# iancze/PSOAP

Hardware: AMD Instinct MI355X
Metric: GP lnprob evals/sec (SB2, N=6000) (higher is better)
Workload: dtype f64; 1 GPU; SB2 chunk 20 epochs x 300 px (N=6000), 32 walkers per step per GPU, one chunk per GPU (BASELINE.json configs[2]; configs[3] at 8 GPUs); timed step = H2D of next proposals || eval, D2H of 32 lnprobs, gather; N=6000, components=2, walkers=32, chunks_per_gpu=1, mode=dag, stream_groups=2, parallelism=chunk-sharded x1, RCCL all_gather of walker lnprobs

## Files before the change

### include/psoap_gp.h

```cpp
#ifndef PSOAP_GP_H
#define PSOAP_GP_H

#include <stdint.h>

#ifdef __cplusplus
extern "C" {
#endif

typedef struct psoap_chunk psoap_chunk;

int psoap_version(void);
const char *psoap_last_error(void);
int psoap_device_count(int *count);

enum {
    PSOAP_SHARE_PROCS = 0,
    PSOAP_SHARE_DAG_LAUNCHES = 1,
    PSOAP_SHARE_TAINTED = 2,
    PSOAP_SHARE_RETRIES = 3,
    PSOAP_SHARE_STAGED_FALLBACKS = 4,
    PSOAP_SHARE_STAGED_POLICY = 5,
    PSOAP_SHARE_MOVED_TASKS = 6,
    PSOAP_SHARE_MOVED_XCD = 7,
    PSOAP_SHARE_LOCK_ACQUISITIONS = 8,
// ... 134 lines not shown
                       long long *tasks_per_matrix);
int psoap_stream_plan(int P, int lanes, int workers, int scheme, void *out, long long max_tasks, long long *n_tasks,
                      long long *n_slots, long long *n_ctrs, int *scheme_out);
int psoap_stream_tasklog(psoap_chunk *h, int cap, unsigned long long *out, long long max_words);
int psoap_stream_tasks(psoap_chunk *h, void *out, long long max_tasks, long long *n_tasks);

int psoap_chunk_dag_tasks(psoap_chunk *h, void *out, long long max_tasks, long long *n_tasks);

int psoap_dag_plan(int B, int P, int workers, void *out, long long max_tasks, long long *n_tasks,
                   long long *n_slots, long long *n_ctrs, unsigned int *queue_first );
int psoap_dag_plan_sky(int B, int P, const int *first, int workers, void *out, long long max_tasks, long long *n_tasks,
                       long long *n_slots, long long *n_ctrs, unsigned int *queue_first );
int psoap_sky_first(int c, int N, int B, const double *lwl, const double *gp, int *first_out, int *perm_out);
int psoap_sky_order(int c, int N, int B, const double *lwl, const double *gp, int *first_out, int *perm_out, int *cand_out);
int psoap_chunk_sky_stats(psoap_chunk *h, long long *out, int n);
int psoap_dag_plan_multi(int B, const int *Ps, int workers, void *out, long long max_tasks,
                         long long *n_tasks, long long *n_slots, long long *n_ctrs,
                         unsigned int *queue_first);
int psoap_dag_plan_aug(int P, int Mt, int Ms, int workers, int scheme, void *tasks_out,
                       long long max_tasks, long long *n_tasks, long long *n_slots,
                       long long *n_ctrs, unsigned int *queue_first);

int psoap_dag_plan_pool(int B, const int *Ps, int workers, int Mt, int Ms, int scheme, void *tasks_out,
                        long long max_tasks, long long *n_tasks, unsigned int *order_out, unsigned int *dep_out,
                        unsigned int *n_main_out, unsigned int *queue_first, int *has_pool, long long *n_ctrs);
int psoap_dag_pick_workers(int B, const int *Ps, int Mt, int compute_units, int max_workers, int *workers);

#ifdef __cplusplus
}
#endif
// ... 2 lines not shown
```

### psoap_amd/_lib.py

```python
from __future__ import annotations

import ctypes
import os

import numpy as np

from .build import LIB_PATH

_dp = ctypes.POINTER(ctypes.c_double)
_ip = ctypes.POINTER(ctypes.c_int)
_i32p = ctypes.POINTER(ctypes.c_int32)
_vp = ctypes.c_void_p

K_CLASSES = 7
K_NAMES = ("fill", "panel_update", "potrf", "trsm", "misc", "dag", "grad_contract")


class Timings(ctypes.Structure):
    _fields_ = [("ms", ctypes.c_double * K_CLASSES),
                ("launches", ctypes.c_int64 * K_CLASSES),
                ("flops", ctypes.c_double * K_CLASSES),
                ("bytes", ctypes.c_double * K_CLASSES),
                ("total_ms", ctypes.c_double)]

# ... 84 lines not shown
    "psoap_chunk_set_profiling": (ctypes.c_int, [_vp, ctypes.c_int]),
    "psoap_chunk_get_timings": (ctypes.c_int, [_vp, ctypes.POINTER(Timings)]),
    "psoap_chunk_set_stream_groups": (ctypes.c_int, [_vp, ctypes.c_int]),
    "psoap_chunk_set_mode": (ctypes.c_int, [_vp, ctypes.c_int]),
    "psoap_chunk_dag_tasklog": (ctypes.c_int, [_vp, ctypes.POINTER(ctypes.c_uint64), ctypes.c_longlong]),
    "psoap_chunk_dag_tasks": (ctypes.c_int, [_vp, _vp, ctypes.c_longlong, ctypes.POINTER(ctypes.c_longlong)]),
    "psoap_dag_plan": (ctypes.c_int, [ctypes.c_int, ctypes.c_int, ctypes.c_int, _vp, ctypes.c_longlong,
                                      ctypes.POINTER(ctypes.c_longlong), ctypes.POINTER(ctypes.c_longlong),
                                      ctypes.POINTER(ctypes.c_longlong), ctypes.POINTER(ctypes.c_uint32)]),
    "psoap_dag_plan_sky": (ctypes.c_int, [ctypes.c_int, ctypes.c_int, _ip, ctypes.c_int, _vp, ctypes.c_longlong,
                                          ctypes.POINTER(ctypes.c_longlong), ctypes.POINTER(ctypes.c_longlong),
                                          ctypes.POINTER(ctypes.c_longlong), ctypes.POINTER(ctypes.c_uint32)]),
    "psoap_sky_first": (ctypes.c_int, [ctypes.c_int, ctypes.c_int, ctypes.c_int, _dp, _dp, _ip, _ip]),
    "psoap_sky_order": (ctypes.c_int, [ctypes.c_int, ctypes.c_int, ctypes.c_int, _dp, _dp, _ip, _ip, _ip]),
    "psoap_chunk_sky_stats": (ctypes.c_int, [_vp, ctypes.POINTER(ctypes.c_longlong), ctypes.c_int]),
    "psoap_dag_plan_multi": (ctypes.c_int, [ctypes.c_int, _ip, ctypes.c_int, _vp, ctypes.c_longlong,
                                      ctypes.POINTER(ctypes.c_longlong), ctypes.POINTER(ctypes.c_longlong),
                                      ctypes.POINTER(ctypes.c_longlong), ctypes.POINTER(ctypes.c_uint32)]),
    "psoap_dag_plan_aug": (ctypes.c_int, [ctypes.c_int, ctypes.c_int, ctypes.c_int, ctypes.c_int, ctypes.c_int, _vp,
                                          ctypes.c_longlong, ctypes.POINTER(ctypes.c_longlong),
                                          ctypes.POINTER(ctypes.c_longlong), ctypes.POINTER(ctypes.c_longlong),
                                          ctypes.POINTER(ctypes.c_uint32)]),
    "psoap_dag_pick_workers": (ctypes.c_int, [ctypes.c_int, _ip, ctypes.c_int, ctypes.c_int, ctypes.c_int, _ip]),
    "psoap_dag_plan_pool": (ctypes.c_int, [ctypes.c_int, _ip, ctypes.c_int, ctypes.c_int, ctypes.c_int, ctypes.c_int, _vp,
                                           ctypes.c_longlong, ctypes.POINTER(ctypes.c_longlong), ctypes.POINTER(ctypes.c_uint32),
                                           ctypes.POINTER(ctypes.c_uint32), ctypes.POINTER(ctypes.c_uint32),
                                           ctypes.POINTER(ctypes.c_uint32), _ip, ctypes.POINTER(ctypes.c_longlong)]),
}

BENCH_SIGNATURES = {
# ... 105 lines not shown
```

### psoap_amd/chunk.py

```python
from __future__ import annotations

import ctypes

import numpy as np

from . import _lib
from ._lib import K_NAMES, Timings, as_f64, check, dptr


class ChunkHandle:
    def __init__(self, fl, sigma, max_batch: int = 1, device: int | None = None):
        self._L = _lib.load()
        self.fl = as_f64(fl)
        self.sigma = as_f64(sigma, self.fl.shape)
        if self.fl.ndim != 1:
            raise ValueError("fl and sigma must be 1-D")
        self.N = int(self.fl.shape[0])
        self.max_batch = int(max_batch)
        self.device = _lib.default_device() if device is None else int(device)
        self._h = ctypes.c_void_p()
        check(self._L.psoap_chunk_create(ctypes.byref(self._h), self.device, self.N, dptr(self.fl),
                                         dptr(self.sigma), self.max_batch), "psoap_chunk_create")
        self._B = 0
        self.n_epochs = 0
# ... 245 lines not shown
        t = Timings()
        check(self._L.psoap_chunk_get_timings(self._h, ctypes.byref(t)), "psoap_chunk_get_timings")
        out = {"total_ms": t.total_ms}
        for k, name in enumerate(K_NAMES):
            out[name] = {"ms": t.ms[k], "launches": int(t.launches[k]), "flops": t.flops[k], "bytes": t.bytes[k]}
        return out

    def sky_stats(self) -> dict:
        names = ("tiles_planned", "tiles_dense", "units_planned", "units_dense", "plan_builds", "cache_hits", "skyline_on")
        out = (ctypes.c_longlong * len(names))()
        n = self._L.psoap_chunk_sky_stats(self._h, out, len(names))
        if n != len(names):
            raise _lib.PsoapError(f"psoap_chunk_sky_stats reports {n} fields, psoap_amd.chunk names {len(names)}")
        return dict(zip(names, (int(v) for v in out)))


class StreamPipeline:

    def __init__(self, handle: ChunkHandle, c: int, walkers: int, groups: int = 2, scheme: int = -1, submit=None):
        if walkers % groups:
            raise ValueError("walkers must be a multiple of groups")
        self.h, self.c, self.walkers, self.groups = handle, int(c), int(walkers), int(groups)
        self.rows = [slice(g * walkers // groups, (g + 1) * walkers // groups) for g in range(groups)]
        handle.stream_open(c, walkers, scheme)
        self._submit = submit if submit is not None else handle.stream_submit
        self.tickets = [None] * groups
        self.period = None

    def _go(self, g, arrays, mu_GP):
        r = self.rows[g]
# ... 109 lines not shown
```

### psoap_amd/csrc/dag_kernel.hpp

```cpp
#pragma once
#include "dag_task.hpp"

#include "chol_kernels.hpp"
#include "fill_kernels.hpp"
#include "potrf_blocked.hpp"
#include "potrf_spine.hpp"
#include "orbit_kernels.hpp"

namespace psoap {

struct alignas(64) MatFlags {
    int rows_done;
    int potrf_done;
    int cnt[2];
    int next_done;
    int off1_ready;
    int step_w[4];
    int cnt3;
    int pad[5];
    int xcol[256][2];
    int rvrow[256];
};
static_assert(sizeof(MatFlags) == 64 + 2048 + 1024, "one cache line of row state + the per-column progress words");

// ... 152 lines not shown
    int* cnt = M3 ? (q % 3 == 2 ? &f->cnt3 : &f->cnt[q % 3]) : &f->cnt[q & 1];
    const int old = __hip_atomic_fetch_add(cnt, n, PSOAP_RLX_AGENT);
    if (old + n == ntasks_row) {
        __builtin_amdgcn_fence(__ATOMIC_ACQ_REL, "agent");
        asm volatile("s_waitcnt vmcnt(0)" ::: "memory");
        __hip_atomic_store(cnt, 0, PSOAP_RLX_AGENT);
        asm volatile("s_waitcnt vmcnt(0)" ::: "memory");
        if (ctl && q > 0) dag_spin_ge(&f->rows_done, q, ctl, 11u);
        __hip_atomic_store(&f->rows_done, q + 1, __ATOMIC_RELEASE, __HIP_MEMORY_SCOPE_AGENT);
    }
}

template <bool SW = false, class SM = SmemKernel, bool ROWMAP = false, bool TD = false>
__device__ __forceinline__ void dag_update(Tile& t, double* Km, int ld, int k0, int j0, int pa, int pb, MatFlags* f,
                                           DagCtl* ctl, bool wait_next, unsigned long long* tl, int wave_s = -1, SM sm = SM(),
                                           int* wa = nullptr, int* wb = nullptr)
{
    if (pb <= pa) return;
    const bool diag = (k0 == j0);
    unsigned long long w0 = 0;
    if (tl && threadIdx.x == 0) w0 = __builtin_amdgcn_s_memrealtime();
    if (pb - pa > 1) {
        if constexpr (TD) dag_wait_ge2(wa, wb, pb - 1, ctl, 1u);
        else dag_wait_ge(&f->rows_done, pb - 1, ctl, 1u);
        if (tl && threadIdx.x == 0) {
            const unsigned long long w1 = __builtin_amdgcn_s_memrealtime();
            tl[7] += (w1 - w0) << 40;
        }
        const size_t r0 = (size_t)pa * NB;
        tile_gemm_tn<SW, SM, ROWMAP>(t, Km + r0 * ld + k0, (size_t)ld, Km + r0 * ld + j0, (size_t)ld, (pb - 1 - pa) * NB, diag, 0x7fffffff, wave_s, sm);
    }
    if (tl && threadIdx.x == 0) w0 = __builtin_amdgcn_s_memrealtime();
    if constexpr (TD) dag_wait_ge2(wa, wb, pb, ctl, 2u);
    else dag_wait_ge(wait_next ? &f->next_done : &f->rows_done, pb, ctl, 2u);
    if (tl && threadIdx.x == 0) {
        const unsigned long long w1 = __builtin_amdgcn_s_memrealtime();
        tl[4] = w1;
        tl[7] += (w1 - w0) << 40;
    }
    const size_t r1 = (size_t)(pb - 1) * NB;
    tile_gemm_tn<SW, SM, ROWMAP>(t, Km + r1 * ld + k0, (size_t)ld, Km + r1 * ld + j0, (size_t)ld, NB, diag, 0x7fffffff, wave_s, sm);
}

template <class SM>
__device__ __forceinline__ void dag_update_following(Tile& t, const double* __restrict__ A, const double* __restrict__ B,
                                                     size_t ld, int* xa, int* xb, int base, unsigned int* err, int wave, SM sm,
                                                     unsigned long long* tl = nullptr)
{
    const int wr = wave >> 1, wc = wave & 1;
    const int lane = hw_lane();
    int avail = ps::x_wait(xa, xb, base, err, 1, lane);
    if (tl && threadIdx.x == 0) tl[4] = __builtin_amdgcn_s_memrealtime();
    __builtin_amdgcn_fence(__ATOMIC_ACQUIRE, "agent");
    stage_glds_w(A, ld, B, ld, 0, 0, wave, sm);
    __syncthreads();
#pragma unroll 1
// ... 25 lines not shown
    const double* rowx;
    const double* diag;
    double* S;
    size_t lds;
};

struct DagMat {
    double* K;
    double* R;
    double* Wt;
    const double* lw;
    const double* gp;
    const double* sigma;
    MatAcc* acc;
    int N, Npad, P, ld;
};

#ifdef PSOAP_FAST_STREAM
#define DAG_FAST_STORE(stream) true
#else
#define DAG_FAST_STORE(stream) (!(stream))
#endif
template <int C, bool AUG, bool INPLACE = false, bool ROWMAP = false, bool FAST = false, bool WT = true>
__device__ __forceinline__ void dag_store_updated(Tile& t, double* __restrict__ dest, size_t ldd, int k0, int j0,
                                                  const double* __restrict__ lw, const GpDev& g, double dsum,
                                                  const double* __restrict__ sigma, int N, double scale,
                                                  int Npad, const DagAug& aug, double* __restrict__ mirror = nullptr,
                                                  bool plain = false)
{
    static_assert(INPLACE || !ROWMAP, "tiles that go to memory use the plain accumulator map");
// ... 1328 lines not shown
#else
        if (LAT && preload && ttype == DAG_DIAG && (task.type & DAG_WAITNEXT) && task.pb - task.pa == 1) {
            dag_diag_fast(Km, ld, k0, Wm, Rv, mat.acc, prev, Npad, f, ctl, q, ntasks_row, (task.type & DAG_FUSED) != 0,
                          &arrive_l[task.ctr], n_wait, dag_opaque_lds(psoap_smem), dag_opaque_lds(vec1), dag_opaque_lds(vec2),
                          tlog_l ? tlog_l + ticket * 8 : nullptr);
            dag_task_end<STREAM>(st, b, mat.acc, mat.P, where0, ctl, wave_s);
            continue;
        }
#endif
        t.zero();
        if (preload) {
            dag_wait_ge(&arrive_l[tctr], n_wait, ctl, 4u);
            dag_sub_partials<false, true>(t, prev, 1);
            n_prev = 0;
        }
        dag_update<true, SmemKernel, false, !LAT && DAG_TILE_DEPS>(
            t, Km, ld, k0, j0, task.pa, task.pb, f, ctl, ttype == DAG_DIAG && (task.type & DAG_WAITNEXT) != 0,
            tlog_l ? tlog_l + ticket * 8 : nullptr, wave_s, SmemKernel(), &f->rvrow[q], &f->rvrow[j]);
        if (tlog_l && threadIdx.x == 0) tlog_l[ticket * 8 + 5] = __builtin_amdgcn_s_memrealtime();
        if (!preload && n_wait > 0) dag_wait_ge(&arrive_l[tctr], n_wait, ctl, 4u);
        if (tlog_l && threadIdx.x == 0) tlog_l[ticket * 8 + 6] = __builtin_amdgcn_s_memrealtime();
        dag_sub_partials<false, true>(t, prev, n_prev);
        {
            GpDev g;
            load_gp(mat.gp, C, g);
            double dsum = g.a2[0];
            {
#pragma clang fp contract(off)
                for (int c = 1; c < C; ++c) dsum = dsum + g.a2[c];
            }
            double* dest = is_part ? (wspace_l + (size_t)task.slot * SLOT) : (Km + (size_t)k0 * ld + j0);
            size_t ldd = is_part ? (size_t)NB : (size_t)ld;
            double* mirror = nullptr;
// ... 82 lines not shown
```

### psoap_amd/csrc/plan_abi.hpp

```cpp
#pragma once
#include <string.h>

#include <algorithm>
#include <vector>

#include "abi_error.hpp"
#include "dag_plan.hpp"
#include "sky_rules.hpp"

using namespace psoap;

static void plan_export(const DagPlan& plan, void* out, long long max_tasks, long long* n_tasks, long long* n_slots,
                        long long* n_ctrs, unsigned int* queue_first)
{
    *n_tasks = (long long)plan.tasks.size();
    if (n_slots) *n_slots = plan.n_slots;
    if (n_ctrs) *n_ctrs = plan.n_ctrs;
    if (queue_first) memcpy(queue_first, plan.queues.first, sizeof plan.queues.first);
    if (out) {
        const long long n = max_tasks < *n_tasks ? max_tasks : *n_tasks;
        memcpy(out, plan.tasks.data(), sizeof(DagTask) * n);
    }
}

// ... 9 lines not shown
                                  long long* n_tasks, long long* n_slots, long long* n_ctrs, unsigned int* queue_first)
{
    if (B < 1 || P < 1 || P > 255 || workers < 1 || !n_tasks || !first) FAIL("psoap_dag_plan_sky: bad arguments");
    bool any = false;
    for (int j = 0; j < P; ++j) {
        if (first[j] < 0 || first[j] > (j > 0 ? j - 1 : 0) || (j > 0 && first[j] < first[j - 1]))
            FAIL("psoap_dag_plan_sky: first must be non-decreasing with 0 <= first[j] <= max(j - 1, 0)");
        any = any || first[j] > 0;
    }
    DagPlan plan = any ? dag_build_tasks(std::vector<int>((size_t)B, P), workers, 0, 0, 0, 0, first) : dag_build_tasks(B, P, workers);
    plan_export(plan, out, max_tasks, n_tasks, n_slots, n_ctrs, queue_first);
    return 0;
}

static long long sky_host_candidate(int c, int N, int B, const double* lwl, const double* gp, int cand, std::vector<int>& perm,
                                    std::vector<int>& first)
{
    const int P = round_up(N, NB) / NB;
    double w[3];
    sky_cand_weights(c, cand, w);
    std::vector<unsigned long long> key((size_t)N);
    for (int i = 0; i < N; ++i) {
        double v[3] = {0.0, 0.0, 0.0};
        for (int k = 0; k < c; ++k) v[k] = lwl[(size_t)k * N + i];
        key[i] = sky_key(sky_cand_key(c, w, v));
    }
    perm.resize((size_t)N);
    first.assign((size_t)P, 0);
    for (int i = 0; i < N; ++i) perm[i] = i;
    std::stable_sort(perm.begin(), perm.end(), [&key](int a, int b) { return key[a] < key[b]; });
    std::vector<double> x((size_t)c * N), lo((size_t)c * P), hi((size_t)c * P);
    std::vector<int> fb((size_t)P);
    for (int b = 0; b < B; ++b) {
        for (int k = 0; k < c; ++k)
            for (int r = 0; r < N; ++r) x[(size_t)k * N + r] = lwl[((size_t)b * c + k) * N + perm[r]];
        for (int k = 0; k < c; ++k)
            for (int t = 0; t < P; ++t)
                sky_interval(x.data() + (size_t)k * N, t * NB, (t + 1) * NB < N ? (t + 1) * NB : N, &lo[(size_t)k * P + t],
                             &hi[(size_t)k * P + t]);
        double p2[3] = {0.0, 0.0, 0.0};
        const bool ok = sky_gp(gp + (size_t)b * 2 * c, c, p2);
        for (int j = 0; j < P; ++j) fb[j] = sky_first_raw(j, P, c, lo.data(), hi.data(), p2, ok);
        sky_first_finish(fb.data(), P);
        for (int j = 0; j < P; ++j) first[j] = (b == 0 || fb[j] < first[j]) ? fb[j] : first[j];
    }
    return sky_cost(first.data(), P);
}

static void sky_host_order(int c, int N, int B, const double* lwl, const double* gp, int n_cand, int* first_out, int* perm_out,
                           int* cand_out)
{
    const int P = round_up(N, NB) / NB;
    std::vector<int> perm((size_t)N), first((size_t)P, 0);
    for (int i = 0; i < N; ++i) perm[i] = i;
    int best = 0;
    if (N <= SKY_MAX_N) {
        long long best_cost = sky_host_candidate(c, N, B, lwl, gp, 0, perm, first);
        std::vector<int> pk, fk;
        for (int k = 1; k < n_cand; ++k) {
            const long long cost = sky_host_candidate(c, N, B, lwl, gp, k, pk, fk);
            if (cost < best_cost) {
                best_cost = cost;
                best = k;
                perm.swap(pk);
                first.swap(fk);
            }
        }
    }
    if (perm_out) memcpy(perm_out, perm.data(), sizeof(int) * (size_t)N);
    if (first_out) memcpy(first_out, first.data(), sizeof(int) * (size_t)P);
    if (cand_out) *cand_out = best;
}

extern "C" int psoap_sky_first(int c, int N, int B, const double* lwl, const double* gp, int* first_out, int* perm_out)
{
    if (c < 1 || c > 3 || N < 1 || B < 1 || !lwl || !gp) FAIL("psoap_sky_first: bad arguments");
    sky_host_order(c, N, B, lwl, gp, 1, first_out, perm_out, nullptr);
    return 0;
}

extern "C" int psoap_sky_order(int c, int N, int B, const double* lwl, const double* gp, int* first_out, int* perm_out,
                               int* cand_out)
{
    if (c < 1 || c > 3 || N < 1 || B < 1 || !lwl || !gp) FAIL("psoap_sky_order: bad arguments");
    sky_host_order(c, N, B, lwl, gp, sky_n_cand(c), first_out, perm_out, cand_out);
    return 0;
}

extern "C" int psoap_stream_plan(int P, int lanes, int workers, int scheme, void* out, long long max_tasks,
                                 long long* n_tasks, long long* n_slots, long long* n_ctrs, int* scheme_out)
{
    if (P < 1 || P > 255 || lanes < 1 || lanes > STREAM_MAX_LANES || workers < 1 || scheme < -1 || scheme > 2 || !n_tasks)
        FAIL("psoap_stream_plan: bad arguments");
    if (scheme < 0) scheme = dag_auto_scheme(std::vector<int>((size_t)lanes, P));
    DagPlan plan = dag_build_lane_plan(P, lanes, workers, scheme);
    plan_export(plan, out, max_tasks, n_tasks, n_slots, n_ctrs, nullptr);
    if (scheme_out) *scheme_out = plan.scheme;
    return 0;
}

// ... 48 lines not shown
```

### psoap_amd/csrc/psoap_gp.hip

```cpp
#include "../../include/psoap_gp.h"

#include <math.h>
#include <stdio.h>
#include <stdlib.h>
#include <stddef.h>
#include <string.h>

#include <errno.h>
#include <time.h>
#include <unistd.h>

#include <algorithm>
#include <atomic>
#include <chrono>
#include <memory>
#include <mutex>
#include <set>
#include <string>
#include <vector>

#include "chol_kernels.hpp"
#include "dag_kernel.hpp"
#include "solo_kernel.hpp"
#include "dag_launch.hpp"
// ... 30 lines not shown
{
    char bus[64] = {0};
    return hipDeviceGetPCIBusId(bus, (int)sizeof bus, device) == hipSuccess ? std::string(bus) : std::string();
}

struct BatchSlot {
    Grow<double> dLwl;
    Grow<double> dGp;
    Grow<double> dLwlS;
    Grow<double> dFlS;
    Grow<double> dSigmaS;
    Grow<int> dPerm;
    Grow<int> dCand;
    Grow<int> dFirstB;
    Grow<int, true> hFirst;
    Grow<int> dTooFast;
    bool toofast_dirty = false;
    Grow<DagMat> dMats;
    int mats_B = 0, mats_C = 0;
    bool mats_sorted = false;
    bool sky_valid = false;
    int B = 0, C = 0;
    double mu = 1.0;
    std::vector<char> neg;
    Event evUpload;
    Event evEval;
};

namespace psoap { struct PredictWs; struct GradWs; }

// ... 44 lines not shown
    Grow<double> dWt;
    Grow<double> dR;
    Grow<MatAcc> dAcc;
    Grow<double> dVel;
    Grow<double> dOut;
    Grow<double> dDates;
    Grow<double> dPorb;
    Grow<double, true> hPorb;
    Grow<unsigned int, true> hDagErr;
    int mode = 1;
    int dag_grid = 0, n_cus = 0;
    DagWorkspace dag;
    int plan_B = 0, plan_workers = 0;
    bool sky = false;
    bool sky_order = true;
    std::vector<int> plan_first;
    DagPlanWork plan_work;
    struct SkyPlan {
        int B;
        std::vector<int> first;
        DagPlan plan;
        int workers;
        DagPlanWork work;
        Grow<DagTask> dTasks;
    };
    std::vector<SkyPlan> sky_cache;
    long long sky_stats[7] = {};
    Grow<unsigned long long> dTlog;
    long long tlog_tasks = 0;
    Grow<double, true> hLwl, hGp, hVel, hOut;
// ... 128 lines not shown
    NEED(h->dWt, nb * WT_STRIDE);
    HIP_TRY(hipMemset(h->dWt, 0, sizeof(double) * nb * WT_STRIDE));
    NEED(h->dR, nb * h->Npad);
    NEED(h->dAcc, ACC_ROWS * nb);
    NEED(h->dOut, nb);
    NEED(h->dPorb, nb * 13);
    NEED(h->hPorb, nb * 13);
    NEED(h->hLwl, nb * 3 * N);
    NEED(h->hGp, nb * 6);
    NEED(h->hOut, nb);
    {
        const char* e = getenv("PSOAP_SKYLINE");
        h->sky = N <= SKY_MAX_N && !(e && e[0] == '0');
        e = getenv("PSOAP_SKY_ORDER");
        h->sky_order = !(e && e[0] == '0');
    }
    const size_t n_cand = h->sky_order ? SKY_MAX_CAND : 1;
    for (BatchSlot& sl : h->slot) {
        if (h->sky) {
            NEED(sl.dLwlS, nb * 3 * N);
            NEED(sl.dFlS, N);
            NEED(sl.dSigmaS, N);
            NEED(sl.dPerm, n_cand * N);
            NEED(sl.dCand, 1);
            HIP_TRY(hipMemset(sl.dCand, 0, sizeof(int)));
            NEED(sl.dFirstB, n_cand * nb * h->P);
            NEED(sl.hFirst, h->P);
            memset(sl.hFirst, 0, sizeof(int) * h->P);
        }
        NEED(sl.dLwl, nb * 3 * N);
        NEED(sl.dGp, nb * 6);
        NEED(sl.dTooFast, nb);
        HIP_TRY(hipMemset(sl.dTooFast, 0, sizeof(int) * nb));
        NEED(sl.dMats, nb);
        HIP_TRY(sl.evUpload.create());
        HIP_TRY(sl.evEval.create());
    }
    const size_t tiles = nb * (size_t)h->P * (h->P + 1) / 2;
    HIP_TRY(h->dag.ctl.need(sizeof(DagCtl) + sizeof(MatFlags) * nb + sizeof(int) * (tiles + 16 + (9 * tiles + 1024) / 32 + 8)));
    NEED(h->hDagErr, 16);
    h->hDagErr[0] = 0;
    if (int rc = dag_workers(h->device, &h->dag_grid, &h->n_cus)) return rc;
// ... 111 lines not shown
    if (out) {
        const long long n = max_tasks < tasks ? max_tasks : tasks;
        HIP_TRY(hipMemcpy(out, h->dTlog, sizeof(unsigned long long) * 8 * n, hipMemcpyDeviceToHost));
    }
    return 0;
}


extern "C" int psoap_chunk_sky_stats(psoap_chunk* h, long long* out, int n)
{
    if (!h || !out || n < 0) FAIL("psoap_chunk_sky_stats: bad arguments");
    for (int i = 0; i < n && i < 7; ++i) out[i] = h->sky_stats[i];
    return 7;
}

extern "C" int psoap_chunk_dag_tasks(psoap_chunk* h, void* out, long long max_tasks, long long* n_tasks)
{
    if (!h || !n_tasks) FAIL("bad arguments");
    DEVICE_SCOPE(h->device);
    if (set_dev(h)) return 1;
    *n_tasks = h->dag.n_tasks;
    if (out && h->dag.tasks) {
        const long long n = max_tasks < (long long)h->dag.n_tasks ? max_tasks : (long long)h->dag.n_tasks;
        HIP_TRY(hipMemcpy(out, h->dag.tasks, sizeof(DagTask) * n, hipMemcpyDeviceToHost));
    }
    return 0;
}

extern "C" int psoap_chunk_set_mode(psoap_chunk* h, int mode)
{
// ... 51 lines not shown
static bool sky_batch(const psoap_chunk* h, int B)
{
    return h->mode == 1 && h->P <= 255 && !dag_fixed_plan() && dag_lnlike_scheme(std::vector<int>((size_t)B, h->P)) == 0;
}

static int upload_end(psoap_chunk* h, BatchSlot& sl)
{
    HIP_TRY(hipMemcpyAsync(sl.dGp, h->hGp, sizeof(double) * (size_t)sl.B * 2 * sl.C, hipMemcpyHostToDevice, h->copy()));
    sl.sky_valid = h->sky && sky_batch(h, sl.B);
    if (sl.sky_valid) {
        const int N = h->N, rows = sl.B * sl.C;
        hipStream_t s = h->copy();
        const int K = h->sky_order ? sky_n_cand(sl.C) : 1;
        hipLaunchKernelGGL(k_sky_perm, dim3((N + 255) / 256, K), dim3(256), 0, s, sl.dLwl, sl.C, N, sl.dPerm);
        hipLaunchKernelGGL(k_sky_first, dim3(sl.B, K), dim3(256), 0, s, sl.dLwl, sl.dPerm, sl.dGp, sl.C, N, h->P, sl.dFirstB);
        hipLaunchKernelGGL(k_sky_choose, dim3(1), dim3(256), 0, s, sl.dFirstB, sl.B, h->P, K, sl.hFirst, sl.dCand);
        hipLaunchKernelGGL(k_sky_gather, dim3((N + 255) / 256, rows + 2), dim3(256), 0, s, sl.dPerm, sl.dCand, N, rows, sl.dLwl,
                           sl.dLwlS, h->dFl, sl.dFlS, h->dSigma, sl.dSigmaS);
        HIP_TRY(hipGetLastError());
    }
    HIP_TRY(hipEventRecord(h->evStaging, h->copy()));
    HIP_TRY(hipEventRecord(sl.evUpload, h->copy()));
    return 0;
}

extern "C" int psoap_batch_upload(psoap_chunk* h, int B, int c, const double* lwl, const double* gp, double mu_GP)
{
    if (!h || !lwl || !gp) FAIL("psoap_batch_upload: bad arguments");
    DEVICE_SCOPE(h->device);
    if (set_dev(h)) return 1;
    BatchSlot* sl = nullptr;
// ... 140 lines not shown
    } else if (int rc = launch()) {
        return rc;
    }
    return prof_end(h, s);
}

template <int C>
static void launch_fill(psoap_chunk* h, const BatchSlot& sl, hipStream_t s, int b0, int nb, int upper_only)
{
    const int tiles = upper_only ? h->P * (h->P + 1) / 2 : h->P * h->P;
    hipLaunchKernelGGL(k_fill_sym<C>, dim3(tiles, nb), dim3(256), 0, s, h->dK + (size_t)b0 * h->mat_stride,
                       h->mat_stride, h->ld, h->N, h->P, sl.dLwl + (size_t)b0 * C * h->N,
                       sl.dGp + (size_t)b0 * 2 * C, h->dSigma, upper_only);
}

static DagMat chunk_mat(const psoap_chunk* h, int b, int C, const double* lw, const double* gp, const double* sigma)
{
    DagMat m{};
    m.K = h->dK + (size_t)b * h->mat_stride;
    m.R = h->dR + (size_t)b * h->Npad;
    m.Wt = h->dWt + (size_t)b * WT_STRIDE;
    m.lw = lw + (size_t)b * C * h->N;
    m.gp = gp + (size_t)b * 2 * C;
    m.sigma = sigma;
    m.acc = h->dAcc + (size_t)b * ACC_ROWS;
    m.N = h->N;
    m.Npad = h->Npad;
    m.P = h->P;
    m.ld = h->ld;
    return m;
}

static void fill_mats(const psoap_chunk* h, const BatchSlot& sl, DagMat* out, bool sorted)
{
    for (int b = 0; b < sl.B; ++b)
        out[b] = chunk_mat(h, b, sl.C, sorted ? sl.dLwlS : sl.dLwl, sl.dGp, sorted ? sl.dSigmaS : h->dSigma);
}

static int promote_slot(psoap_chunk* h, const char* who)
{
    if (h->pend >= 0) {
        h->act = h->pend;
        h->pend = -1;
    }
    if (h->act < 0 || h->slot[h->act].B < 1) {
        g_err = std::string(who) + ": nothing uploaded";
        return 2;
    }
    return 0;
}

// ... 119 lines not shown
    HIP_TRY(hipEventRecord(h->evLast, s));
    h->last_recorded = true;
    HIP_TRY(hipMemcpyAsync(h->hOut, h->dOut, sizeof(double) * sl.B, hipMemcpyDeviceToHost, s));
    HIP_TRY(hipMemcpyAsync(h->hDagErr, &ctl->error, 6 * sizeof(unsigned int), hipMemcpyDeviceToHost, s));
    h->last_path = 1;
    return 0;
}

static int eval_dag(psoap_chunk* h)
{
    BatchSlot& sl = h->slot[h->act];
    const int B = sl.B, C = sl.C, N = h->N, P = h->P;
    hipStream_t s = h->streams[0];
    h->recs.clear();
    if (int rc = dag_prepare(h)) return rc;
    HIP_TRY(hipStreamWaitEvent(s, sl.evUpload, 0));
    if (int rc = prof_launch(h, s, PSOAP_K_MISC, 0.0, 0.0, [&]() -> int {
        hipLaunchKernelGGL(k_init_rhs, dim3((h->Npad + 255) / 256, B), dim3(256), 0, s, h->dR, h->Npad, N,
                           h->plan_first.empty() ? h->dFl.p : sl.dFlS.p, sl.mu, h->dAcc);
        HIP_TRY(hipGetLastError());
        HIP_TRY(hipMemsetAsync(h->dag.ctl, 0, h->dag.ctl_bytes, s));
        static const int poison = getenv("PSOAP_DEBUG_POISON") ? atoi(getenv("PSOAP_DEBUG_POISON")) : 0;
        if (poison & 1) HIP_TRY(hipMemsetAsync(h->dK, 0xFF, sizeof(double) * h->mat_stride * (size_t)B, s));
        if (poison & 2)
            for (int b = 0; b < B; ++b)
                HIP_TRY(hipMemsetAsync(h->dWt + (size_t)b * WT_STRIDE + (size_t)2 * NB * NB, 0xFF, sizeof(double) * MB_DOUBLES, s));
        if ((poison & 4) && h->dag.n_slots) HIP_TRY(hipMemsetAsync(h->dag.ws, 0xFF, sizeof(double) * NB * NB * (size_t)h->dag.n_slots, s));
        if (poison & 8) HIP_TRY(hipMemsetAsync(h->dAcc, 0xFF, sizeof(MatAcc) * ACC_ROWS * (size_t)B, s));
        return 0;
        })) return rc;
// ... 4 lines not shown
        return rc;
    if (int rc = dag_tail(h, s, h->dag.dag_ctl(), true)) return rc;
    g_share.dag_launches += 1;
    return 0;
}

static int eval_staged(psoap_chunk* h);

extern "C" int psoap_batch_eval(psoap_chunk* h)
{
    if (!h) FAIL("psoap_batch_eval: null handle");
    DEVICE_SCOPE(h->device);
    if (set_dev(h)) return 1;
    if (int rc = promote_slot(h, "psoap_batch_eval")) return rc;
    h->last_group = nullptr;
    if (int rc = handle_lock(h)) return rc;
    int rc;
    if (h->mode == 1 && h->P <= 255 && !share_wants_staged(h->device)) {
        rc = eval_dag(h);
    } else {
        if (h->mode == 1 && h->P <= 255) g_share.staged_policy += 1;
        rc = eval_staged(h);
    }
    if (rc) handle_unlock(h);
    return rc;
}

static int eval_staged(psoap_chunk* h)
{
    h->last_path = 0;
// ... 218 lines not shown
        const BatchSlot& sl = h->slot[h->act];
        HIP_TRY(hipStreamWaitEvent(s, sl.evUpload, 0));
        hipLaunchKernelGGL(k_init_rhs, dim3((h->Npad + 255) / 256, sl.B), dim3(256), 0, s, h->dR, h->Npad, h->N, h->dFl,
                           sl.mu, h->dAcc);
        h->recs.clear();
    }
    HIP_TRY(hipGetLastError());
    HIP_TRY(hipMemsetAsync(g->dag.ctl, 0, g->dag.ctl_bytes, s));
    int Pmax_g = 0;
    for (psoap_chunk* h : g->hs) Pmax_g = h->P > Pmax_g ? h->P : Pmax_g;
    launch_lnlike(g->hs[0], g->dag, g->workers, C, g->dMats, total, Pmax_g, s, nullptr);
    HIP_TRY(hipGetLastError());
    for (psoap_chunk* h : g->hs) {
        if (int rc = dag_tail(h, s, g->dag.dag_ctl(), false)) return rc;
        h->last_group = g;
    }
    g_share.dag_launches += 1;
    HIP_TRY(hipGetLastError());
    HIP_TRY(hipEventRecord(g->evDone, s));
    for (psoap_chunk* h : g->hs) HIP_TRY(hipStreamWaitEvent(h->streams[0], g->evDone, 0));
    return 0;
}

extern "C" int psoap_group_stats(psoap_group* g, long long* plan_builds, long long* record_refreshes)
{
    if (!g) FAIL("psoap_group_stats: null group");
    if (plan_builds) *plan_builds = g->plan_builds;
    if (record_refreshes) *record_refreshes = g->record_refreshes;
    return 0;
}
// ... 1131 lines not shown
```

### psoap_amd/csrc/sky_kernels.hpp

```cpp
#pragma once
#include "common.hpp"
#include "sky_rules.hpp"

namespace psoap {

__global__ __launch_bounds__(256) void k_sky_perm(const double* __restrict__ x, int C, int N, int* __restrict__ perm)
{
    __shared__ unsigned long long keys[1024];
    const int cand = blockIdx.y;
    double w[3];
    sky_cand_weights(C, cand, w);
    auto key = [&](int i) {
        double v[3] = {0.0, 0.0, 0.0};
        for (int c = 0; c < C; ++c) v[c] = x[(size_t)c * N + i];
        return sky_key(sky_cand_key(C, w, v));
    };
    const int i = blockIdx.x * 256 + threadIdx.x;
    const unsigned long long mine = i < N ? key(i) : 0ull;
    int rank = 0;
    for (int k0 = 0; k0 < N; k0 += 1024) {
        __syncthreads();
        for (int k = threadIdx.x; k < 1024; k += 256) keys[k] = k0 + k < N ? key(k0 + k) : ~0ull;
        __syncthreads();
#pragma unroll 16
// ... 49 lines not shown
            lo[idx] = nan ? -__builtin_inf() : a;
            hi[idx] = nan ? __builtin_inf() : z;
        }
    }
    __syncthreads();
    double p2[3] = {0.0, 0.0, 0.0};
    const bool ok = sky_gp(gp + (size_t)b * 2 * C, C, p2);
    if ((int)threadIdx.x < P) fb[threadIdx.x] = sky_first_raw((int)threadIdx.x, P, C, lo, hi, p2, ok);
    __syncthreads();
    if (threadIdx.x == 0) sky_first_finish(fb, P);
    __syncthreads();
    if ((int)threadIdx.x < P) first_b[((size_t)cand * B + b) * P + threadIdx.x] = fb[threadIdx.x];
}

__global__ __launch_bounds__(256) void k_sky_choose(const int* __restrict__ first_b, int B, int P, int K,
                                                    int* __restrict__ first_host, int* __restrict__ cand_out)
{
    __shared__ int fu[SKY_MAX_CAND * SKY_MAX_P];
    __shared__ long long cost[SKY_MAX_CAND];
    __shared__ int win;
    for (int idx = threadIdx.x; idx < K * P; idx += 256) {
        const int k = idx / P, j = idx % P;
        const int* f = first_b + (size_t)k * B * P + j;
        int m = f[0];
        for (int b = 1; b < B; ++b) m = f[(size_t)b * P] < m ? f[(size_t)b * P] : m;
        fu[idx] = m;
    }
    __syncthreads();
    if ((int)threadIdx.x < K) cost[threadIdx.x] = sky_cost(fu + threadIdx.x * P, P);
    __syncthreads();
    if (threadIdx.x == 0) {
        int best = 0;
        for (int k = 1; k < K; ++k) best = cost[k] < cost[best] ? k : best;
        win = best;
        cand_out[0] = best;
    }
    __syncthreads();
    for (int j = threadIdx.x; j < P; j += 256) first_host[j] = fu[win * P + j];
}

}
```

### psoap_amd/csrc/sky_rules.hpp

```cpp
#pragma once
#include "tile_consts.hpp"

namespace psoap {

constexpr int SKY_MAX_N = 8192;
constexpr int SKY_MAX_P = SKY_MAX_N / NB;
constexpr int SKY_MAX_CAND = 15;

PSOAP_HD inline unsigned long long sky_key(double x)
{
    const unsigned long long u = __builtin_bit_cast(unsigned long long, x);
    return (u >> 63) ? ~u : (u | 0x8000000000000000ull);
}

PSOAP_HD inline int sky_n_cand(int C) { return C == 2 ? 9 : C == 3 ? 15 : 1; }

PSOAP_HD inline void sky_cand_weights(int C, int k, double* w)
{
    w[0] = 1.0;
    w[1] = w[2] = 0.0;
    if (C == 2) {
        w[0] = 1.0 - k / 8.0;
        w[1] = k / 8.0;
    } else if (C == 3) {
// ... 20 lines not shown
        any = true;
    }
    return acc;
}

PSOAP_HD inline long long sky_cost(const int* first, int P)
{
    long long u = 0;
    for (int j = 0; j < P; ++j) {
        const long long d = j - first[j];
        u += d * (d + 1) / 2;
    }
    return u;
}

PSOAP_HD inline bool sky_gp(const double* gp, int C, double* p2)
{
#pragma clang fp contract(off)
    bool ok = true;
    for (int c = 0; c < C; ++c) {
        const double amp = gp[2 * c], l = gp[2 * c + 1];
        const double a2 = amp * amp;
        if (!(amp > 0.0 && a2 < __builtin_inf() && l > 0.0 && l < __builtin_inf())) ok = false;
        p2[c] = -0.5 * (C_KMS * C_KMS) / (l * l);
    }
    return ok;
}

PSOAP_HD inline void sky_interval(const double* x, int i0, int i1, double* lo, double* hi)
{
// ... 44 lines not shown
```

Baseline: 1719 evals/s.

## Clip DAG panel-update GEMM ranges to each matrix's per-batch skyline start

The skyline plan uses a first-nonzero row per column that is the minimum across all walkers in the batch. The change keeps each walker's own first-nonzero tile table, copied from the winning candidate in k_sky_choose, and passes it to the DAG update. There each matrix's trailing GEMM starts at max(pa, first_b[j]) and skips tiles known to be zero. This cuts redundant FLOPs for walkers whose kernel is sparser than the batch minimum, at the cost of an extra device copy, a scalar read per task and possible load imbalance between workers. Stats helpers are added to count the clipped units.

```diff
diff --git a/include/psoap_gp.h b/include/psoap_gp.h
--- a/include/psoap_gp.h
+++ b/include/psoap_gp.h
@@ -172,6 +172,10 @@
 int psoap_sky_first(int c, int N, int B, const double *lwl, const double *gp, int *first_out, int *perm_out);
 int psoap_sky_order(int c, int N, int B, const double *lwl, const double *gp, int *first_out, int *perm_out, int *cand_out);
 int psoap_chunk_sky_stats(psoap_chunk *h, long long *out, int n);
+int psoap_sky_first_b(int c, int N, int B, const double *lwl, const double *gp, int *first_b_out, int *cand_out);
+int psoap_sky_clip_units(int B, int P, const int *first, const int *first_b, int workers, long long *units,
+                         long long *tiles_empty);
+int psoap_chunk_sky_clip_stats(psoap_chunk *h, const int *first_b, int B, long long *out, int n);
 int psoap_dag_plan_multi(int B, const int *Ps, int workers, void *out, long long max_tasks,
                          long long *n_tasks, long long *n_slots, long long *n_ctrs,
                          unsigned int *queue_first);
diff --git a/psoap_amd/_lib.py b/psoap_amd/_lib.py
--- a/psoap_amd/_lib.py
+++ b/psoap_amd/_lib.py
@@ -122,6 +122,10 @@
     "psoap_sky_first": (ctypes.c_int, [ctypes.c_int, ctypes.c_int, ctypes.c_int, _dp, _dp, _ip, _ip]),
     "psoap_sky_order": (ctypes.c_int, [ctypes.c_int, ctypes.c_int, ctypes.c_int, _dp, _dp, _ip, _ip, _ip]),
     "psoap_chunk_sky_stats": (ctypes.c_int, [_vp, ctypes.POINTER(ctypes.c_longlong), ctypes.c_int]),
+    "psoap_sky_first_b": (ctypes.c_int, [ctypes.c_int, ctypes.c_int, ctypes.c_int, _dp, _dp, _ip, _ip]),
+    "psoap_sky_clip_units": (ctypes.c_int, [ctypes.c_int, ctypes.c_int, _ip, _ip, ctypes.c_int,
+                                            ctypes.POINTER(ctypes.c_longlong), ctypes.POINTER(ctypes.c_longlong)]),
+    "psoap_chunk_sky_clip_stats": (ctypes.c_int, [_vp, _ip, ctypes.c_int, ctypes.POINTER(ctypes.c_longlong), ctypes.c_int]),
     "psoap_dag_plan_multi": (ctypes.c_int, [ctypes.c_int, _ip, ctypes.c_int, _vp, ctypes.c_longlong,
                                       ctypes.POINTER(ctypes.c_longlong), ctypes.POINTER(ctypes.c_longlong),
                                       ctypes.POINTER(ctypes.c_longlong), ctypes.POINTER(ctypes.c_uint32)]),
diff --git a/psoap_amd/chunk.py b/psoap_amd/chunk.py
--- a/psoap_amd/chunk.py
+++ b/psoap_amd/chunk.py
@@ -283,6 +283,24 @@
             raise _lib.PsoapError(f"psoap_chunk_sky_stats reports {n} fields, psoap_amd.chunk names {len(names)}")
         return dict(zip(names, (int(v) for v in out)))
 
+    def sky_clip_stats(self, lwl, gp) -> dict:
+        lwl = np.ascontiguousarray(lwl, dtype=np.float64)
+        gp = np.ascontiguousarray(gp, dtype=np.float64)
+        B, c, N = lwl.shape
+        if N != self.N or gp.shape != (B, 2 * c):
+            raise ValueError(f"sky_clip_stats: lwl (B, c, {self.N}) and gp (B, 2c) of the evaluated batch")
+        ip = ctypes.POINTER(ctypes.c_int)
+        first_b = np.zeros((B, (N + 127) // 128), dtype=np.int32)
+        check(self._L.psoap_sky_first_b(c, N, B, lwl.ctypes.data_as(ctypes.POINTER(ctypes.c_double)),
+                                        gp.ctypes.data_as(ctypes.POINTER(ctypes.c_double)), first_b.ctypes.data_as(ip), None),
+              "psoap_sky_first_b")
+        names = ("units_clipped", "tiles_empty", "clip_on")
+        out = (ctypes.c_longlong * len(names))()
+        n = self._L.psoap_chunk_sky_clip_stats(self._h, first_b.ctypes.data_as(ip), B, out, len(names))
+        if n != len(names):
+            check(n, "psoap_chunk_sky_clip_stats")
+        return dict(zip(names, (int(v) for v in out)))
+
 
 class StreamPipeline:
 
diff --git a/psoap_amd/csrc/dag_kernel.hpp b/psoap_amd/csrc/dag_kernel.hpp
--- a/psoap_amd/csrc/dag_kernel.hpp
+++ b/psoap_amd/csrc/dag_kernel.hpp
@@ -6,6 +6,7 @@
 #include "potrf_blocked.hpp"
 #include "potrf_spine.hpp"
 #include "orbit_kernels.hpp"
+#include "sky_rules.hpp"
 
 namespace psoap {
 
@@ -190,9 +191,10 @@
 template <bool SW = false, class SM = SmemKernel, bool ROWMAP = false, bool TD = false>
 __device__ __forceinline__ void dag_update(Tile& t, double* Km, int ld, int k0, int j0, int pa, int pb, MatFlags* f,
                                            DagCtl* ctl, bool wait_next, unsigned long long* tl, int wave_s = -1, SM sm = SM(),
-                                           int* wa = nullptr, int* wb = nullptr)
+                                           int* wa = nullptr, int* wb = nullptr, int ps = -1)
 {
     if (pb <= pa) return;
+    if (ps < 0) ps = pa;
     const bool diag = (k0 == j0);
     unsigned long long w0 = 0;
     if (tl && threadIdx.x == 0) w0 = __builtin_amdgcn_s_memrealtime();
@@ -203,8 +205,9 @@
             const unsigned long long w1 = __builtin_amdgcn_s_memrealtime();
             tl[7] += (w1 - w0) << 40;
         }
-        const size_t r0 = (size_t)pa * NB;
-        tile_gemm_tn<SW, SM, ROWMAP>(t, Km + r0 * ld + k0, (size_t)ld, Km + r0 * ld + j0, (size_t)ld, (pb - 1 - pa) * NB, diag, 0x7fffffff, wave_s, sm);
+        const size_t r0 = (size_t)ps * NB;
+        if (pb - 1 > ps)
+            tile_gemm_tn<SW, SM, ROWMAP>(t, Km + r0 * ld + k0, (size_t)ld, Km + r0 * ld + j0, (size_t)ld, (pb - 1 - ps) * NB, diag, 0x7fffffff, wave_s, sm);
     }
     if (tl && threadIdx.x == 0) w0 = __builtin_amdgcn_s_memrealtime();
     if constexpr (TD) dag_wait_ge2(wa, wb, pb, ctl, 2u);
@@ -215,7 +218,8 @@
         tl[7] += (w1 - w0) << 40;
     }
     const size_t r1 = (size_t)(pb - 1) * NB;
-    tile_gemm_tn<SW, SM, ROWMAP>(t, Km + r1 * ld + k0, (size_t)ld, Km + r1 * ld + j0, (size_t)ld, NB, diag, 0x7fffffff, wave_s, sm);
+    if (pb > ps)
+        tile_gemm_tn<SW, SM, ROWMAP>(t, Km + r1 * ld + k0, (size_t)ld, Km + r1 * ld + j0, (size_t)ld, NB, diag, 0x7fffffff, wave_s, sm);
 }
 
 template <class SM>
@@ -271,6 +275,7 @@
     const double* sigma;
     MatAcc* acc;
     int N, Npad, P, ld;
+    const int* first_b;
 };
 
 #ifdef PSOAP_FAST_STREAM
@@ -1629,9 +1634,13 @@
             dag_sub_partials<false, true>(t, prev, 1);
             n_prev = 0;
         }
+        int ps = -1;
+        if constexpr (SKY) {
+            if (mat.first_b) ps = sky_clip_start((int)task.pa, (int)task.pb, __builtin_amdgcn_readfirstlane(mat.first_b[j]));
+        }
         dag_update<true, SmemKernel, false, !LAT && DAG_TILE_DEPS>(
             t, Km, ld, k0, j0, task.pa, task.pb, f, ctl, ttype == DAG_DIAG && (task.type & DAG_WAITNEXT) != 0,
-            tlog_l ? tlog_l + ticket * 8 : nullptr, wave_s, SmemKernel(), &f->rvrow[q], &f->rvrow[j]);
+            tlog_l ? tlog_l + ticket * 8 : nullptr, wave_s, SmemKernel(), &f->rvrow[q], &f->rvrow[j], ps);
         if (tlog_l && threadIdx.x == 0) tlog_l[ticket * 8 + 5] = __builtin_amdgcn_s_memrealtime();
         if (!preload && n_wait > 0) dag_wait_ge(&arrive_l[tctr], n_wait, ctl, 4u);
         if (tlog_l && threadIdx.x == 0) tlog_l[ticket * 8 + 6] = __builtin_amdgcn_s_memrealtime();
diff --git a/psoap_amd/csrc/plan_abi.hpp b/psoap_amd/csrc/plan_abi.hpp
--- a/psoap_amd/csrc/plan_abi.hpp
+++ b/psoap_amd/csrc/plan_abi.hpp
@@ -47,7 +47,7 @@
 }
 
 static long long sky_host_candidate(int c, int N, int B, const double* lwl, const double* gp, int cand, std::vector<int>& perm,
-                                    std::vector<int>& first)
+                                    std::vector<int>& first, std::vector<int>* first_b = nullptr)
 {
     const int P = round_up(N, NB) / NB;
     double w[3];
@@ -64,6 +64,7 @@
     std::stable_sort(perm.begin(), perm.end(), [&key](int a, int b) { return key[a] < key[b]; });
     std::vector<double> x((size_t)c * N), lo((size_t)c * P), hi((size_t)c * P);
     std::vector<int> fb((size_t)P);
+    if (first_b) first_b->assign((size_t)B * P, 0);
     for (int b = 0; b < B; ++b) {
         for (int k = 0; k < c; ++k)
             for (int r = 0; r < N; ++r) x[(size_t)k * N + r] = lwl[((size_t)b * c + k) * N + perm[r]];
@@ -76,30 +77,33 @@
         for (int j = 0; j < P; ++j) fb[j] = sky_first_raw(j, P, c, lo.data(), hi.data(), p2, ok);
         sky_first_finish(fb.data(), P);
         for (int j = 0; j < P; ++j) first[j] = (b == 0 || fb[j] < first[j]) ? fb[j] : first[j];
+        if (first_b) std::copy(fb.begin(), fb.end(), first_b->begin() + (size_t)b * P);
     }
     return sky_cost(first.data(), P);
 }
 
 static void sky_host_order(int c, int N, int B, const double* lwl, const double* gp, int n_cand, int* first_out, int* perm_out,
-                           int* cand_out)
+                           int* cand_out, int* first_b_out = nullptr)
 {
     const int P = round_up(N, NB) / NB;
-    std::vector<int> perm((size_t)N), first((size_t)P, 0);
+    std::vector<int> perm((size_t)N), first((size_t)P, 0), table((size_t)B * P, 0);
     for (int i = 0; i < N; ++i) perm[i] = i;
     int best = 0;
     if (N <= SKY_MAX_N) {
-        long long best_cost = sky_host_candidate(c, N, B, lwl, gp, 0, perm, first);
-        std::vector<int> pk, fk;
+        long long best_cost = sky_host_candidate(c, N, B, lwl, gp, 0, perm, first, first_b_out ? &table : nullptr);
+        std::vector<int> pk, fk, tk;
         for (int k = 1; k < n_cand; ++k) {
-            const long long cost = sky_host_candidate(c, N, B, lwl, gp, k, pk, fk);
+            const long long cost = sky_host_candidate(c, N, B, lwl, gp, k, pk, fk, first_b_out ? &tk : nullptr);
             if (cost < best_cost) {
                 best_cost = cost;
                 best = k;
                 perm.swap(pk);
                 first.swap(fk);
+                table.swap(tk);
             }
         }
     }
+    if (first_b_out) memcpy(first_b_out, table.data(), sizeof(int) * (size_t)B * P);
     if (perm_out) memcpy(perm_out, perm.data(), sizeof(int) * (size_t)N);
     if (first_out) memcpy(first_out, first.data(), sizeof(int) * (size_t)P);
     if (cand_out) *cand_out = best;
@@ -117,6 +121,50 @@
 {
     if (c < 1 || c > 3 || N < 1 || B < 1 || !lwl || !gp) FAIL("psoap_sky_order: bad arguments");
     sky_host_order(c, N, B, lwl, gp, sky_n_cand(c), first_out, perm_out, cand_out);
+    return 0;
+}
+
+extern "C" int psoap_sky_first_b(int c, int N, int B, const double* lwl, const double* gp, int* first_b_out, int* cand_out)
+{
+    if (c < 1 || c > 3 || N < 1 || B < 1 || !lwl || !gp || !first_b_out) FAIL("psoap_sky_first_b: bad arguments");
+    sky_host_order(c, N, B, lwl, gp, sky_n_cand(c), nullptr, nullptr, cand_out, first_b_out);
+    return 0;
+}
+
+static void sky_clip_count(const std::vector<DagTask>& tasks, int B, int P, const int* first_b, long long* units,
+                           long long* tiles_empty)
+{
+    std::vector<int> planned((size_t)B * P * P, 0), left((size_t)B * P * P, 0);
+    long long u = 0, e = 0;
+    for (const DagTask& t : tasks) {
+        if ((int)t.b >= B || (int)t.q >= P || (int)t.j >= P) continue;
+        const int pa = t.pa, pb = t.pb;
+        const int ps = first_b ? sky_clip_start(pa, pb, first_b[(size_t)t.b * P + t.j]) : pa;
+        const size_t at = ((size_t)t.b * P + t.q) * P + t.j;
+        planned[at] += pb > pa ? pb - pa : 0;
+        left[at] += pb > ps ? pb - ps : 0;
+    }
+    for (size_t at = 0; at < planned.size(); ++at) {
+        u += left[at];
+        e += (planned[at] > 0 && left[at] == 0) ? 1 : 0;
+    }
+    *units = u;
+    *tiles_empty = e;
+}
+
+extern "C" int psoap_sky_clip_units(int B, int P, const int* first, const int* first_b, int workers, long long* units,
+                                    long long* tiles_empty)
+{
+    if (B < 1 || P < 1 || P > 255 || workers < 1 || !first || !first_b || !units || !tiles_empty)
+        FAIL("psoap_sky_clip_units: bad arguments");
+    bool any = false;
+    for (int j = 0; j < P; ++j) {
+        if (first[j] < 0 || first[j] > (j > 0 ? j - 1 : 0) || (j > 0 && first[j] < first[j - 1]))
+            FAIL("psoap_sky_clip_units: first must be non-decreasing with 0 <= first[j] <= max(j - 1, 0)");
+        any = any || first[j] > 0;
+    }
+    const DagPlan plan = any ? dag_build_tasks(std::vector<int>((size_t)B, P), workers, 0, 0, 0, 0, first) : dag_build_tasks(B, P, workers);
+    sky_clip_count(plan.tasks, B, P, first_b, units, tiles_empty);
     return 0;
 }
 
diff --git a/psoap_amd/csrc/psoap_gp.hip b/psoap_amd/csrc/psoap_gp.hip
--- a/psoap_amd/csrc/psoap_gp.hip
+++ b/psoap_amd/csrc/psoap_gp.hip
@@ -68,6 +68,7 @@
     Grow<int> dCand;
     Grow<int> dFirstB;
     Grow<int, true> hFirst;
+    Grow<int> dClip;
     Grow<int> dTooFast;
     bool toofast_dirty = false;
     Grow<DagMat> dMats;
@@ -142,6 +143,8 @@
     int plan_B = 0, plan_workers = 0;
     bool sky = false;
     bool sky_order = true;
+    bool sky_clip = true;
+    bool clip_ran = false;
     std::vector<int> plan_first;
     DagPlanWork plan_work;
     struct SkyPlan {
@@ -300,6 +303,8 @@
         h->sky = N <= SKY_MAX_N && !(e && e[0] == '0');
         e = getenv("PSOAP_SKY_ORDER");
         h->sky_order = !(e && e[0] == '0');
+        e = getenv("PSOAP_SKY_CLIP");
+        h->sky_clip = !(e && e[0] == '0');
     }
     const size_t n_cand = h->sky_order ? SKY_MAX_CAND : 1;
     for (BatchSlot& sl : h->slot) {
@@ -312,6 +317,8 @@
             HIP_TRY(hipMemset(sl.dCand, 0, sizeof(int)));
             NEED(sl.dFirstB, n_cand * nb * h->P);
             NEED(sl.hFirst, h->P);
+            NEED(sl.dClip, nb * h->P);
+            HIP_TRY(hipMemset(sl.dClip, 0, sizeof(int) * nb * h->P));
             memset(sl.hFirst, 0, sizeof(int) * h->P);
         }
         NEED(sl.dLwl, nb * 3 * N);
@@ -453,6 +460,22 @@
     return 7;
 }
 
+extern "C" int psoap_chunk_sky_clip_stats(psoap_chunk* h, const int* first_b, int B, long long* out, int n)
+{
+    if (!h || !out || n < 0) FAIL("psoap_chunk_sky_clip_stats: bad arguments");
+    long long v[3] = {h->sky_stats[2], 0, 0};
+    if (h->clip_ran && !h->plan_first.empty() && h->plan_B > 0) {
+        if (!first_b || B != h->plan_B) FAIL("psoap_chunk_sky_clip_stats: first_b (B, P) of the batch evaluated last is needed");
+        size_t at = 0;
+        while (at < h->sky_cache.size() && !(h->sky_cache[at].B == h->plan_B && h->sky_cache[at].first == h->plan_first)) ++at;
+        if (at == h->sky_cache.size()) FAIL("psoap_chunk_sky_clip_stats: the list of the last evaluation is no longer cached");
+        sky_clip_count(h->sky_cache[at].plan.tasks, B, h->P, first_b, &v[0], &v[1]);
+        v[2] = 1;
+    }
+    for (int i = 0; i < n && i < 3; ++i) out[i] = v[i];
+    return 3;
+}
+
 extern "C" int psoap_chunk_dag_tasks(psoap_chunk* h, void* out, long long max_tasks, long long* n_tasks)
 {
     if (!h || !n_tasks) FAIL("bad arguments");
@@ -534,7 +557,8 @@
         const int K = h->sky_order ? sky_n_cand(sl.C) : 1;
         hipLaunchKernelGGL(k_sky_perm, dim3((N + 255) / 256, K), dim3(256), 0, s, sl.dLwl, sl.C, N, sl.dPerm);
         hipLaunchKernelGGL(k_sky_first, dim3(sl.B, K), dim3(256), 0, s, sl.dLwl, sl.dPerm, sl.dGp, sl.C, N, h->P, sl.dFirstB);
-        hipLaunchKernelGGL(k_sky_choose, dim3(1), dim3(256), 0, s, sl.dFirstB, sl.B, h->P, K, sl.hFirst, sl.dCand);
+        hipLaunchKernelGGL(k_sky_choose, dim3(1), dim3(256), 0, s, sl.dFirstB, sl.B, h->P, K, sl.hFirst, sl.dCand,
+                           sl.dClip);
         hipLaunchKernelGGL(k_sky_gather, dim3((N + 255) / 256, rows + 2), dim3(256), 0, s, sl.dPerm, sl.dCand, N, rows, sl.dLwl,
                            sl.dLwlS, h->dFl, sl.dFlS, h->dSigma, sl.dSigmaS);
         HIP_TRY(hipGetLastError());
@@ -705,7 +729,8 @@
                        sl.dGp + (size_t)b0 * 2 * C, h->dSigma, upper_only);
 }
 
-static DagMat chunk_mat(const psoap_chunk* h, int b, int C, const double* lw, const double* gp, const double* sigma)
+static DagMat chunk_mat(const psoap_chunk* h, int b, int C, const double* lw, const double* gp, const double* sigma,
+                        const int* clip = nullptr)
 {
     DagMat m{};
     m.K = h->dK + (size_t)b * h->mat_stride;
@@ -719,13 +744,15 @@
     m.Npad = h->Npad;
     m.P = h->P;
     m.ld = h->ld;
+    m.first_b = clip ? clip + (size_t)b * h->P : nullptr;
     return m;
 }
 
 static void fill_mats(const psoap_chunk* h, const BatchSlot& sl, DagMat* out, bool sorted)
 {
     for (int b = 0; b < sl.B; ++b)
-        out[b] = chunk_mat(h, b, sl.C, sorted ? sl.dLwlS : sl.dLwl, sl.dGp, sorted ? sl.dSigmaS : h->dSigma);
+        out[b] = chunk_mat(h, b, sl.C, sorted ? sl.dLwlS : sl.dLwl, sl.dGp, sorted ? sl.dSigmaS : h->dSigma,
+                           sorted && h->sky_clip ? sl.dClip.p : nullptr);
 }
 
 static int promote_slot(psoap_chunk* h, const char* who)
@@ -875,6 +902,7 @@
     hipStream_t s = h->streams[0];
     h->recs.clear();
     if (int rc = dag_prepare(h)) return rc;
+    h->clip_ran = h->sky_clip && !h->plan_first.empty();
     HIP_TRY(hipStreamWaitEvent(s, sl.evUpload, 0));
     if (int rc = prof_launch(h, s, PSOAP_K_MISC, 0.0, 0.0, [&]() -> int {
         hipLaunchKernelGGL(k_init_rhs, dim3((h->Npad + 255) / 256, B), dim3(256), 0, s, h->dR, h->Npad, N,
@@ -909,6 +937,7 @@
     if (set_dev(h)) return 1;
     if (int rc = promote_slot(h, "psoap_batch_eval")) return rc;
     h->last_group = nullptr;
+    h->clip_ran = false;
     if (int rc = handle_lock(h)) return rc;
     int rc;
     if (h->mode == 1 && h->P <= 255 && !share_wants_staged(h->device)) {
@@ -1157,6 +1186,7 @@
     for (psoap_chunk* h : g->hs) {
         if (int rc = dag_tail(h, s, g->dag.dag_ctl(), false)) return rc;
         h->last_group = g;
+        h->clip_ran = false;
     }
     g_share.dag_launches += 1;
     HIP_TRY(hipGetLastError());
diff --git a/psoap_amd/csrc/sky_kernels.hpp b/psoap_amd/csrc/sky_kernels.hpp
--- a/psoap_amd/csrc/sky_kernels.hpp
+++ b/psoap_amd/csrc/sky_kernels.hpp
@@ -87,7 +87,8 @@
 }
 
 __global__ __launch_bounds__(256) void k_sky_choose(const int* __restrict__ first_b, int B, int P, int K,
-                                                    int* __restrict__ first_host, int* __restrict__ cand_out)
+                                                    int* __restrict__ first_host, int* __restrict__ cand_out,
+                                                    int* __restrict__ clip)
 {
     __shared__ int fu[SKY_MAX_CAND * SKY_MAX_P];
     __shared__ long long cost[SKY_MAX_CAND];
@@ -110,6 +111,7 @@
     }
     __syncthreads();
     for (int j = threadIdx.x; j < P; j += 256) first_host[j] = fu[win * P + j];
+    for (int idx = threadIdx.x; idx < B * P; idx += 256) clip[idx] = first_b[(size_t)win * B * P + idx];
 }
 
 }
diff --git a/psoap_amd/csrc/sky_rules.hpp b/psoap_amd/csrc/sky_rules.hpp
--- a/psoap_amd/csrc/sky_rules.hpp
+++ b/psoap_amd/csrc/sky_rules.hpp
@@ -58,6 +58,12 @@
     return u;
 }
 
+PSOAP_HD inline int sky_clip_start(int pa, int pb, int fb)
+{
+    const int m = fb < pb ? fb : pb;
+    return pa > m ? pa : m;
+}
+
 PSOAP_HD inline bool sky_gp(const double* gp, int C, double* p2)
 {
 #pragma clang fp contract(off)
```

Result: faster. 1836 evals/s (median of 6 runs) (+6.8%).
